# rmcolq/charon

Hardware: AMD Instinct MI355X
Metric: classified reads/sec + achieved HBM GB/s vs roofline, 5 kb reads, 39 GB index (higher is better)
Workload: dtype u64

## Files before the change

### charon_amd/csrc/charon_hip.hip

```cpp

#include <hip/hip_runtime.h>

#include <algorithm>
#include <chrono>
#include <functional>
#include <cmath>
#include <cstddef>
#include <cstdint>
#include <cstdio>
#include <cstdlib>
#include <cstring>
#include <limits>
#include <mutex>
#include <new>
#include <string>
#include <type_traits>
#include <vector>

#include "charon_hip.h"
#include "default_kde.inc"

#include "parts/common.inc"
#include "parts/k1_minimise_probe.inc"
#include "parts/k2_count_wavelog.inc"
#include "parts/shard_kernels.inc"
#include "parts/shardx_kernels.inc"
#include "parts/k3_model_call.inc"
#include "parts/len_order.inc"
#include "parts/gzip_trees.inc"
#include "parts/gzip_walk.inc"
#include "parts/gzip_tally.inc"
#include "parts/gzip_size_dev.inc"
#include "parts/gzip_tally_long.inc"
#include "parts/text_pack.inc"
#include "parts/text_split.inc"
#include "parts/fasta_split.inc"
#include "parts/text_gather.inc"
// ... 20 lines not shown
```

### charon_amd/csrc/parts/abi_shard_wait.inc

```

static int ensure_shard_buffers(chn_stream *s) {
    const uint64_t nw = (s->cfg.max_reads + WAVE - 1) / WAVE;
    int rc;
    if ((rc = s->big.ensure(s->cfg.max_bases, nw, (uint32_t)s->idx->d.bin_words, 65536, 0))) return rc;
    if ((rc = s->d_list.ensure(s->big.log_cap * 8)) || (rc = s->d_cbase.ensure((nw + 1) * 8))) return rc;
    return CHN_OK;
}
static ShardArgs shard_args(chn_stream *s, const chn_index *shard, uint64_t *partial, const Slot &sl) {
    ShardArgs a;
    std::memset(&a, 0, sizeof a);
    const chn_index_desc &d = shard->d;
    a.list = s->d_list.as<uint64_t>(); a.wave_meta = s->big.meta.as<WaveMeta>(); a.cbase = s->d_cbase.as<uint64_t>();
    a.wave_count = s->big.wcount.as<uint32_t>(); a.words = shard->words; a.S = d.bin_size; a.row_begin = d.row_begin; a.row_end = d.row_end;
    a.shift = (uint32_t)d.hash_shift; a.h = d.hash_funs; a.W = (uint32_t)d.bin_words; a.partial = partial; a.rows = s->big.rows.as<uint64_t>();
    a.rowlog = s->big.log.as<uint32_t>(); a.B = (uint32_t)d.bins;
    a.n_waves = (uint32_t)((sl.n_reads + WAVE - 1) / WAVE); a.esc_capacity = s->big.esc_cap;
    a.status = reinterpret_cast<uint32_t *>(const_cast<Slot &>(sl).d_ctl.as<unsigned long long>() + CTL_STATUS);
    return a;
}

extern "C" int chn_shard_minimise(chn_stream *s, const chn_batch *b, uint64_t *n_entries) {
    if (!s || !b || !n_entries) return fail(CHN_E_INVALID, "chn_shard_minimise: null argument");
    if (s->shard_open || s->shx_stage != 0) return fail(CHN_E_STATE, "chn_shard_minimise: previous sharded batch not finished");
    HIPCHK(hipSetDevice(s->idx->d.device));
// ... 125 lines not shown
    const chn_index_desc &d = s->idx->d;
    unsigned long long *ctl = sl.d_ctl.as<unsigned long long>();
    const uint64_t n = sl.n_reads, nw = (n + WAVE - 1) / WAVE + sl.split_bound;
    HIPCHK(hipMemsetAsync(ctl, 0, CTL_NLONG * 8, s->stream));
    HIPCHK(hipMemsetAsync(ctl + CTL_FETCHES, 0, (CTL_WORDS - CTL_FETCHES) * 8, s->stream));
    hipLaunchKernelGGL(k_sum_len, dim3((uint32_t)std::min<uint64_t>(1024, (n + 255) / 256)), dim3(256), 0, s->stream, sl.len1, sl.len2, (uint32_t)n, ctl + CTL_WORDS - 1);
    HIPCHK(hipGetLastError());
    unsigned long long total = 0;
    HIPCHK(hipMemcpyAsync(&total, ctl + CTL_WORDS - 1, 8, hipMemcpyDeviceToHost, s->stream));
    HIPCHK(hipStreamSynchronize(s->stream));
    int rc = s->big.ensure(total, (n + WAVE - 1) / WAVE + std::min<uint64_t>(sl.split_bound, total / len_bucket_floor(std::min(s->long_bucket, 247u)) + 1), (uint32_t)d.bin_words, 65536, 0, nw);
    if (rc) return rc;
    K1Args a = sl.k1;
    a.gate_started = a.gate_signal = nullptr;
    fill_k1_log(a, sl, s->big, true);
    const size_t lds = k1_lds_bytes(a.wn, d.num_categories, MODE_ROWS, a.h, (uint32_t)d.bin_words, (uint32_t)d.bins);
    hipError_t e = launch_k1_mode(MODE_ROWS, (uint32_t)d.bin_words, a, lds, s->stream);
    if (e == hipSuccess && sl.split_bound) e = launch_k1_split_mode(MODE_ROWS, (uint32_t)d.bin_words, a, lds, s->stream, split_grid(sl.split_bound));
    if (e != hipSuccess) return fail(CHN_E_HIP, std::string("k_minimise_probe re-run: ") + hipGetErrorString(e));
    if ((rc = launch_tail(s, sl, s->big, s->stream))) return rc;
    HIPCHK(hipStreamSynchronize(s->stream));
    s->overflow_reruns += 1;
    return CHN_OK;
}

extern "C" int chn_batch_wait(chn_stream *s, chn_result *r) {
    if (!s || !r || r->struct_size != sizeof(chn_result)) return fail(CHN_E_INVALID, "chn_batch_wait: bad argument");
    if (s->inflight == 0) return fail(CHN_E_STATE, "no batch in flight");
    HIPCHK(hipSetDevice(s->idx->d.device));
    Slot &sl = s->slot[(s->head + chn_stream::N_SLOTS - s->inflight) % chn_stream::N_SLOTS];
    static const bool diag_wait = diag_env("CHN_DIAG_WAIT") != nullptr;
// ... 227 lines not shown
```

### charon_amd/csrc/parts/abi_stream_batch.inc

```

struct ResLayout {
    size_t ctl, prob, nh, counts, unique, call, conf, flags, total;
    ResLayout(uint64_t n, uint64_t C) {
        ctl = 0; prob = CTL_WORDS * 8; nh = prob + n * C * 8; counts = nh + n * 4; unique = counts + n * C * 4; call = unique + n * C * 4;
        conf = call + n; flags = conf + n; total = flags + n;
    }
};

static const int PROF_ANCHOR_SECONDS = 8;
static hipError_t prof_anchor_now(chn_stream *s) {
    for (Slot &sl : s->slot) sl.new_anchor = false;
    s->prof_cur = 0; s->prof_anchor_pending = false; s->prof_have_end = false; s->prof_prev_end = 0;
    hipError_t e = hipEventRecord(s->prof_anchor[0], s->stream);
    if (e == hipSuccess) e = hipEventSynchronize(s->prof_anchor[0]);
    s->prof_anchor_at = std::chrono::steady_clock::now();
    return e;
}

extern "C" int chn_stream_create(chn_index *idx, const chn_stream_cfg *cfg, chn_stream **out) {
    if (!idx || !cfg || !out || cfg->struct_size != sizeof(chn_stream_cfg)) return fail(CHN_E_INVALID, "chn_stream_create: bad argument");
    if (cfg->max_reads == 0 || cfg->max_reads > 0xFFFFFF00ULL) return fail(CHN_E_INVALID, "max_reads out of range");
    HIPCHK(hipSetDevice(idx->d.device));
    idx->ef_release();
    chn_stream *s = new (std::nothrow) chn_stream();
// ... 183 lines not shown
    k.memo = s->d_memo.as<ulonglong2>(); k.memo_mask = memo_entries - 1;
    k.tab = s->d_model.as<uint32_t>();
    k.data = reinterpret_cast<const float *>(static_cast<char *>(s->d_model.p) + tab_bytes);
    k.C = C; k.h_pos = M.h_pos; k.h_neg = M.h_neg; k.rate = M.rate; k.log_rate = std::log(M.rate);
    k.min_quality = M.min_quality; k.min_compression = M.min_compression; k.cpt = M.cpt; k.lo_thr = M.lo_thr;
    k.min_pd = M.min_pd; k.min_prd = M.min_prd; k.min_length = M.min_length; k.conf_thr = (int32_t)M.conf_thr;
    k.min_hits = M.min_hits; k.paired = M.paired; k.host_index = M.host_index;
    k.dist = M.dist;
    k.dparams = reinterpret_cast<const float *>(static_cast<char *>(s->d_model.p) + tab_bytes + flat_bytes);
    s->k3 = k;
    s->model = std::move(M);
    s->model.set = true;
    return CHN_OK;
}

static bool k1_cond(int mode, uint32_t B) { return mode == MODE_FUSED && B <= K1_COND_MAX_BINS; }
template <int W, int MODE, bool SPLIT = false, bool COND = false>
static hipError_t launch_k1(const K1Args &a, size_t lds, hipStream_t st, uint32_t blocks = 0) {
    if (!SPLIT) blocks = (a.n_reads + WAVE - 1) / WAVE;
    if (lds > 48 * 1024) {
        hipError_t e = hipFuncSetAttribute((const void *)k_minimise_probe<W, MODE, 0, SPLIT, COND>, hipFuncAttributeMaxDynamicSharedMemorySize, (int)lds);
        if (e != hipSuccess) return e;
    }
    if (a.wn == 23)
        hipLaunchKernelGGL((k_minimise_probe<W, MODE, 23, SPLIT, COND>), dim3(blocks), dim3(WAVE), lds, st, a);
    else
        hipLaunchKernelGGL((k_minimise_probe<W, MODE, 0, SPLIT, COND>), dim3(blocks), dim3(WAVE), lds, st, a);
    return hipGetLastError();
}
static hipError_t launch_k1_split_mode(int mode, uint32_t W, const K1Args &a, size_t lds, hipStream_t st, uint32_t blocks) {
    if (mode == MODE_FUSED) return k1_cond(mode, a.B) ? launch_k1<1, MODE_FUSED, true, true>(a, lds, st, blocks) : launch_k1<1, MODE_FUSED, true, false>(a, lds, st, blocks);
    switch (W) {
        case 1: return launch_k1<1, MODE_ROWS, true>(a, lds, st, blocks);
        case 2: return launch_k1<2, MODE_ROWS, true>(a, lds, st, blocks);
        case 3: return launch_k1<3, MODE_ROWS, true>(a, lds, st, blocks);
        default: return launch_k1<4, MODE_ROWS, true>(a, lds, st, blocks);
    }
}
static uint32_t split_bound(const chn_stream *s, const Slot &sl, uint64_t n, uint64_t n_bases, bool paired) {
// ... 2 lines not shown
    (void)n_bases;
    if (!sl.host_batch) return (uint32_t)n;
    uint64_t c = 0;
    for (uint32_t L : sl.h_len1) c += L >= floor_len;
    return (uint32_t)c;
}
static uint32_t split_grid(uint32_t bound) { return std::min<uint32_t>(bound, 8192u); }
template <int MODE>
static hipError_t launch_k1_w(uint32_t W, const K1Args &a, size_t lds, hipStream_t st) {
    switch (W) {
        case 1: return launch_k1<1, MODE>(a, lds, st);
        case 2: return launch_k1<2, MODE>(a, lds, st);
        case 3: return launch_k1<3, MODE>(a, lds, st);
        default: return launch_k1<4, MODE>(a, lds, st);
    }
}
static size_t k1_lds_bytes(uint32_t wn, uint32_t C, int mode, uint32_t h, uint32_t W, uint32_t B) {
    const bool cond = k1_cond(mode, B);
    const size_t qc = cond ? QCAP + WAVE : QCAP;
    size_t b = (size_t)wn * WAVE * 8 + qc * 8 + qc * 4 + (cond ? qc * 8 : 0) + (mode == MODE_EMPLACE ? WAVE * 8 : 0) + (size_t)wn * WAVE;
    if (mode == MODE_FUSED) b += (size_t)2 * C * WAVE * 4;
    if (cond) b += (size_t)FUSED_ROUNDS * 1024;
    else if (mode == MODE_FUSED || mode == MODE_ROWS) b += (size_t)2 * h * (W <= 2 ? 1 : 2) * 1024;
    b = (b + 15) & ~(size_t)15;
    if (mode == MODE_ROWS) b += (size_t)(CHN_LOG_BATCH + 1) * WAVE * 4;
    return b;
}

static int upload(DevBuf &buf, const void *src, size_t bytes, hipStream_t st, size_t reserve = 0) {
    int rc = buf.ensure(std::max<size_t>(std::max(bytes, reserve), 16));
    if (rc) return rc;
    if (bytes) HIPCHK(hipMemcpyAsync(buf.p, src, bytes, hipMemcpyHostToDevice, st));
    return CHN_OK;
}

static int launch_tail(chn_stream *s, Slot &sl, LogBuf &lb, hipStream_t st);
static void fill_k1_log(K1Args &a, Slot &sl, LogBuf &lb, bool dynamic) {
    a.rowlog = lb.log.as<uint32_t>(); a.rows = lb.rows.as<uint64_t>(); a.wave_meta = lb.meta.as<WaveMeta>(); a.wave_count = lb.wcount.as<uint32_t>();
    a.log_capacity = lb.log_cap; a.esc_capacity = lb.esc_cap; a.cap_num = lb.cap_num; a.esc_shift = lb.esc_shift;
    a.cursor = dynamic ? sl.d_ctl.as<unsigned long long>() + CTL_LOG_CURSOR : nullptr;
}
// ... 257 lines not shown
    dt[2] = dnow();
    unsigned long long *ctl = sl.d_ctl.as<unsigned long long>();
    hipLaunchKernelGGL(k_len_hist, dim3(LEN_BLOCKS), dim3(256), 0, s->stream0, sl.len1, sl.len2, (uint32_t)n, s->d_hist.as<uint32_t>(), ctl);
    sl.split_bound = list_mode ? 0u : split_bound(s, sl, n, b->n_bases, paired);
    hipLaunchKernelGGL(k_len_scatter, dim3(LEN_BLOCKS), dim3(256), 0, s->stream0, sl.len1, sl.len2, (uint32_t)n, s->d_hist.as<uint32_t>(), sl.d_order.as<uint32_t>(),
                       ctl, sl.split_bound ? s->long_bucket : 256u, sl.split_bound);
    HIPCHK(hipGetLastError());
    HIPCHK(hipEventRecord(sl.uploaded, s->stream0));
    HIPCHK(hipStreamWaitEvent(ps, sl.uploaded, 0));

    K1Args &a = sl.k1;
    std::memset(&a, 0, sizeof(a));
    a.words = s->idx->words; a.S = d.bin_size; a.row_begin = d.row_begin; a.row_end = d.row_end; a.seed = d.minimiser_seed; a.powk1 = pow5(d.kmer_size - 1);
    a.shift = (uint32_t)d.hash_shift; a.h = d.hash_funs; a.k = d.kmer_size; a.wn = d.window_size - d.kmer_size + 1;
    a.n_reads = (uint32_t)n; a.nseg = paired ? 2 : 1; a.B = (uint32_t)d.bins; a.C = C;
    for (uint32_t bb = 0; bb < 8 && bb < d.bins; ++bb) a.b2c_packed |= (uint64_t)d.bin_to_category[bb] << (8 * bb);
    a.bases = bases; a.nmask = nmask; a.off1 = off1; a.off2 = off2; a.len1 = sl.len1; a.len2 = sl.len2; a.n_bases = b->n_bases;
    a.order = sl.d_order.as<uint32_t>();
    a.status = reinterpret_cast<uint32_t *>(ctl + CTL_STATUS);
    if (const char *ab = diag_env("CHN_ABLATE")) a.ablate = (uint32_t)std::atoi(ab);
    a.nt_probes = s->idx->rows_local * d.bin_words * 8 > (4ULL << 30) ? 1u : 0u;
    if (const char *nt = diag_env("CHN_NT_PROBES")) a.nt_probes = (uint32_t)std::atoi(nt);
    a.num_hashes = sl.d_num_hashes.as<uint32_t>(); a.counts = sl.d_counts.as<uint32_t>(); a.unique = sl.d_unique.as<uint32_t>();
    const uint32_t n_waves = (uint32_t)((n + WAVE - 1) / WAVE);
    a.n_long_ptr = sl.split_bound ? ctl + CTL_NLONG : nullptr; a.wave_slot0 = n_waves;
    a.fetches = ctl + CTL_FETCHES;
    if (list_kind == LIST_SPARSE) {
        fill_k1_log(a, sl, s->shx, true);
        a.rows = s->d_list.as<uint64_t>();
    } else if (list_mode) {
        fill_k1_log(a, sl, s->big, false);
        a.rows = s->d_list.as<uint64_t>();
        hipLaunchKernelGGL(k_wave_caps, dim3((uint32_t)((n + 255) / 256)), dim3(256), 0, ps, sl.d_order.as<uint32_t>(), sl.len1, sl.len2,
                           (uint32_t)n, s->big.cap_num, s->big.esc_shift, s->big.meta.as<WaveMeta>());
        hipLaunchKernelGGL(k_scan_meta, dim3(1), dim3(1024), 0, ps, s->big.meta.as<WaveMeta>(), n_waves);
        HIPCHK(hipGetLastError());
    } else if (!fused) {
        fill_k1_log(a, sl, sl.lb, true);
    }
    const int mode = list_mode ? MODE_LIST : fused ? MODE_FUSED : MODE_ROWS;
    size_t lds = k1_lds_bytes(a.wn, C, mode, a.h, W, a.B);
    if (const char *pad = diag_env("CHN_LDS_PAD")) lds += (size_t)std::atoi(pad);
    if (lds > 160 * 1024) return fail(CHN_E_INVALID, "window too large for LDS");
    if (sl.split_bound) {
        HIPCHK(hipStreamWaitEvent(s->stream4, sl.uploaded, 0));
        hipError_t e4 = launch_k1_split_mode(mode, W, a, lds, s->stream4, split_grid(sl.split_bound));
        if (e4 != hipSuccess) return fail(CHN_E_HIP, std::string("k_minimise_probe (split) launch: ") + hipGetErrorString(e4));
        HIPCHK(hipEventRecord(sl.split_done, s->stream4));
    }
    const bool gated = !list_mode && alternate && s->gate_signal != nullptr;
    if (gated) {
        if (s->gate_seq) {
            HIPCHK(hipStreamWaitValue64(ps, s->gate_signal, s->gate_seq, hipStreamWaitValueGte, ~0ull));
            s->gated_batches += 1;
        }
        a.gate_started = ctl + CTL_GATE; a.gate_signal = s->gate_signal; a.gate_value = s->gate_seq + 1;
// ... 38 lines not shown
    const uint32_t W = (uint32_t)d.bin_words, C = d.num_categories;
    const uint32_t n_waves = (uint32_t)((n + WAVE - 1) / WAVE);
    const bool prof = (s->cfg.flags & CHN_STREAM_PROFILE) != 0 && st == s->stream2;
    unsigned long long *ctl = sl.d_ctl.as<unsigned long long>();
    if (!sl.fused) {
        K2Args k2;
        std::memset(&k2, 0, sizeof(k2));
        k2.rows = lb.rows.as<uint64_t>(); k2.rowlog = lb.log.as<uint32_t>();
        k2.wave_meta = lb.meta.as<WaveMeta>(); k2.wave_count = lb.wcount.as<uint32_t>(); k2.order = sl.d_order.as<uint32_t>();
        k2.counts = sl.d_counts.as<uint32_t>(); k2.unique = sl.d_unique.as<uint32_t>();
        k2.n_reads = (uint32_t)n; k2.B = (uint32_t)d.bins; k2.C = C; k2.W = W;
        std::memcpy(k2.b2c, d.bin_to_category, 256);
        k2.n_long_ptr = sl.split_bound && !sl.list_mode ? ctl + CTL_NLONG : nullptr; k2.wave_slot0 = n_waves;
        const dim3 grid(n_waves), block(K2_THREADS);
        const bool t16 = !sl.list_mode && sl.len2 == nullptr && s->long_bucket <= LONG_BUCKET_DEFAULT;
        uint32_t G = WAVE;
        while (G > 8 && k2_lds_bytes((uint32_t)d.bins, C, W, G, t16) > K2_LDS_BUDGET) G >>= 1;
        k2.group = G;
        const size_t lds2 = k2_lds_bytes((uint32_t)d.bins, C, W, G, t16);
        if (lds2 > 150 * 1024) return fail(CHN_E_INVALID, "bins x categories too large for the count kernel's LDS");
        const void *fn = t16 ? (W == 1 ? (const void *)k_count_wavelog<1, true> : W == 2 ? (const void *)k_count_wavelog<2, true> : W == 3 ? (const void *)k_count_wavelog<3, true> : (const void *)k_count_wavelog<4, true>)
                             : (W == 1 ? (const void *)k_count_wavelog<1, false> : W == 2 ? (const void *)k_count_wavelog<2, false> : W == 3 ? (const void *)k_count_wavelog<3, false> : (const void *)k_count_wavelog<4, false>);
        if (lds2 > 48 * 1024) HIPCHK(hipFuncSetAttribute(fn, hipFuncAttributeMaxDynamicSharedMemorySize, (int)lds2));
        if (prof) HIPCHK(hipEventRecord(sl.ev[2], st));
        {
            void *args[] = {(void *)&k2};
            HIPCHK(hipLaunchKernel(fn, grid, block, args, lds2, st));
        }
        if (k2.n_long_ptr) {
            const dim3 lgrid(std::min<uint32_t>(sl.split_bound, 4096u)), lblock(K2L_THREADS);
            switch (W) {
                case 1: hipLaunchKernelGGL(k_count_longlog<1>, lgrid, lblock, 0, st, k2); break;
// ... 60 lines not shown
```

### charon_amd/csrc/parts/abi_synth_memory.inc

```

extern "C" int chn_synth_genomes(int device, uint64_t seed, uint64_t n_genomes, uint64_t genome_len, uint32_t **dev_bases2) {
    if (!dev_bases2 || genome_len % 64 || n_genomes == 0) return fail(CHN_E_INVALID, "chn_synth_genomes: bad argument");
    HIPCHK(hipSetDevice(device));
    const uint64_t nd = n_genomes * genome_len / 16;
    uint32_t *p = nullptr;
    HIPCHK(hipMalloc((void **)&p, nd * 4));
    hipLaunchKernelGGL(k_synth_genomes, dim3((uint32_t)std::min<uint64_t>(65535, (nd + 255) / 256)), dim3(256), 0, 0, p, nd, seed);
    HIPCHK(hipGetLastError());
    HIPCHK(hipDeviceSynchronize());
    *dev_bases2 = p;
    return CHN_OK;
}
template <int W, int NT, int U>
__global__ __launch_bounds__(256) void k_gather_roof(const uint64_t *words, uint64_t rows, uint32_t iters, uint64_t *sink) {
    extern __shared__ unsigned char roof_lds[];
    uint64_t s = (blockIdx.x * (uint64_t)blockDim.x + threadIdx.x) * 0x9E3779B97F4A7C15ULL + 1;
    uint64_t acc = 0;
    typedef unsigned long long ull2 __attribute__((ext_vector_type(2)));
    for (uint32_t it = 0; it < iters; it += U) {
        ull2 v[U];
        uint64_t v1[U];
#pragma unroll
        for (int u = 0; u < U; ++u) {
            uint64_t z = s + 0x9E3779B97F4A7C15ULL;
// ... 80 lines not shown
    HIPCHK(hipMalloc((void **)&len, n * 4));
    HIPCHK(hipMalloc((void **)&bin, n));
    std::vector<uint8_t> hb(n);
    for (uint64_t i = 0; i < n; ++i) {
        hb[i] = genome_bin[i / cpg];
        if (hb[i] >= d.bins) { (void)hipFree(off); (void)hipFree(len); (void)hipFree(bin); return fail(CHN_E_INVALID, "genome_bin out of range"); }
    }
    HIPCHK(hipMemcpy(bin, hb.data(), n, hipMemcpyHostToDevice));
    hipLaunchKernelGGL(k_chunk_layout, dim3((uint32_t)((n + 255) / 256)), dim3(256), 0, 0, n_genomes, genome_len, chunk, overlap, cpg, off, len);
    K1Args a;
    std::memset(&a, 0, sizeof(a));
    a.words = idx->words; a.words_rw = idx->words; a.S = d.bin_size; a.row_begin = d.row_begin; a.row_end = d.row_end; a.seed = d.minimiser_seed; a.powk1 = pow5(d.kmer_size - 1);
    a.shift = (uint32_t)d.hash_shift; a.h = d.hash_funs; a.k = d.kmer_size; a.wn = d.window_size - d.kmer_size + 1;
    a.n_reads = (uint32_t)n; a.nseg = 1; a.B = (uint32_t)d.bins; a.C = d.num_categories;
    a.bases = dev_bases2; a.off1 = off; a.len1 = len; a.read_bin = bin; a.n_bases = n_genomes * genome_len;
    const size_t lds = k1_lds_bytes(a.wn, d.num_categories, MODE_EMPLACE, a.h, (uint32_t)d.bin_words, (uint32_t)d.bins);
    hipError_t e = launch_k1_w<MODE_EMPLACE>((uint32_t)d.bin_words, a, lds, 0);
    if (e == hipSuccess) e = hipDeviceSynchronize();
    (void)hipFree(off); (void)hipFree(len); (void)hipFree(bin);
    if (e != hipSuccess) return fail(CHN_E_HIP, std::string("plant: ") + hipGetErrorString(e));
    return CHN_OK;
}
extern "C" int chn_synth_reads(int device, uint64_t seed, const uint32_t *dev_genomes, uint64_t n_genomes, uint64_t genome_len,
                               uint64_t first_read_id, uint64_t n_reads, uint32_t read_len_min, uint32_t read_len_max, double sub_rate, double random_fraction,
                               float mean_quality, chn_synth_reads_out *out) {
    if (!out || n_reads == 0 || read_len_min == 0 || read_len_max < read_len_min) return fail(CHN_E_INVALID, "chn_synth_reads: bad argument");
    if (n_genomes && (!dev_genomes || genome_len < read_len_max)) return fail(CHN_E_INVALID, "genomes shorter than reads");
    HIPCHK(hipSetDevice(device));
    std::memset(out, 0, sizeof(*out));
    uint64_t *d_total = nullptr;
    HIPCHK(hipMalloc((void **)&out->seg1_length, n_reads * 4));
// ... 67 lines not shown
```

### charon_amd/csrc/parts/k1_minimise_probe.inc

```

enum { MODE_FUSED = 0, MODE_ROWS = 1, MODE_EMPLACE = 2, MODE_LIST = 3 };
#ifndef CHN_LOG_BATCH
#define CHN_LOG_BATCH 4
#endif
#ifndef CHN_BASE_PIECES
#define CHN_BASE_PIECES 4
#endif

#ifndef K1_COND_MAX_BINS
#define K1_COND_MAX_BINS 4u
#endif
#ifndef FUSED_ROUNDS
#define FUSED_ROUNDS 2u
#endif

struct WaveMeta { uint64_t base, esc_base; uint32_t cap, esc_cap, pad0, pad1; };

struct K1Args {
    const uint64_t *words;
    uint64_t *words_rw;
    uint64_t S, row_begin, row_end, seed, powk1;
    uint32_t shift, h, k, wn, n_reads, nseg, B, C;
    uint64_t b2c_packed;
    const uint32_t *bases, *nmask;
// ... 1 lines not shown
    const uint32_t *len1, *len2;
    const uint32_t *order;
    uint32_t *num_hashes, *counts, *unique;
    uint64_t *rows;
    uint32_t *rowlog;
    WaveMeta *wave_meta;
    uint32_t *wave_count;
    unsigned long long *cursor;
    uint64_t log_capacity, esc_capacity;
    uint32_t cap_num, esc_shift;
    uint32_t *status;
    uint64_t n_bases;
    uint32_t nt_probes;
    const uint8_t *read_bin;
    uint32_t ablate;
    const unsigned long long *n_long_ptr;
    uint32_t wave_slot0;
    unsigned long long *fetches;
    unsigned long long *gate_started, *gate_signal;
    unsigned long long gate_value;
};
__global__ void k_gate_release(unsigned long long *signal, unsigned long long value) {
    if (threadIdx.x == 0 && blockIdx.x == 0) [[clang::atomic(remote_memory, fine_grained_memory)]] {
        (void)__hip_atomic_fetch_max(signal, value, __ATOMIC_RELAXED, __HIP_MEMORY_SCOPE_SYSTEM);
    }
}

__device__ bool first_window_tied(const K1Args &a, uint64_t o, uint32_t wn) {
    const uint64_t INV5 = 0xCCCCCCCCCCCCCCCDULL;
    const uint32_t k = a.k, w = wn + k - 1;
// ... 63 lines not shown
    switch (n) {
        case 0: asm volatile("s_waitcnt vmcnt(0)" ::: "memory"); break;
        case 1: asm volatile("s_waitcnt vmcnt(1)" ::: "memory"); break;
        case 2: asm volatile("s_waitcnt vmcnt(2)" ::: "memory"); break;
        case 3: asm volatile("s_waitcnt vmcnt(3)" ::: "memory"); break;
        case 4: asm volatile("s_waitcnt vmcnt(4)" ::: "memory"); break;
        case 5: asm volatile("s_waitcnt vmcnt(5)" ::: "memory"); break;
        case 6: asm volatile("s_waitcnt vmcnt(6)" ::: "memory"); break;
        case 7: asm volatile("s_waitcnt vmcnt(6)" ::: "memory"); break;
        case 8: asm volatile("s_waitcnt vmcnt(8)" ::: "memory"); break;
        case 9: asm volatile("s_waitcnt vmcnt(8)" ::: "memory"); break;
        default: asm volatile("s_waitcnt vmcnt(10)" ::: "memory"); break;
    }
}

template <int W, int MODE, int WN_T, bool SPLIT = false, bool COND_T = false>
__global__ __launch_bounds__(WAVE) void k_minimise_probe(const K1Args a) {
    extern __shared__ __align__(16) unsigned char smem[];
    if (!SPLIT && a.gate_started && threadIdx.x == 0) {
        if (atomicAdd(a.gate_started, 1ULL) == (unsigned long long)gridDim.x - 1) [[clang::atomic(remote_memory, fine_grained_memory)]] {
            (void)__hip_atomic_fetch_max(a.gate_signal, a.gate_value, __ATOMIC_RELAXED, __HIP_MEMORY_SCOPE_SYSTEM);
        }
    }
    const uint32_t n_long = a.n_long_ptr ? (uint32_t)__builtin_nontemporal_load(a.n_long_ptr) : 0u;
    uint32_t item = blockIdx.x;
    if (SPLIT && item >= n_long) return;
    do {
    const uint32_t wslot = SPLIT ? a.wave_slot0 + item : item;
    const uint32_t wn = WN_T ? (uint32_t)WN_T : a.wn;
    constexpr uint32_t NBLK = (W == 1 || W == 2) ? 1u : 2u;
// ... 2 lines not shown
    auto qwrap = [&](uint32_t x) -> uint32_t {
        if (!COND) return x & (QC - 1);
        x = x >= QC ? x - QC : x;
        return x >= QC ? x - QC : x;
    };
    const uint32_t pb_round = COND ? 1024u : (MODE == MODE_FUSED || MODE == MODE_ROWS) ? a.h * NBLK * 1024u : 0u;
    unsigned char *pbuf = smem;
    const uint32_t pbuf_lds = (uint32_t)(size_t)(__attribute__((address_space(3))) unsigned char *)smem;
    uint64_t *ring = reinterpret_cast<uint64_t *>(smem + (COND ? FUSED_ROUNDS : 2u) * pb_round);
    uint64_t *qv = ring + (size_t)wn * WAVE;
    uint64_t *qa = qv + QC;
    uint32_t *qm = reinterpret_cast<uint32_t *>(qa + (COND ? QC : 0u));
    uint64_t *rbase = reinterpret_cast<uint64_t *>(qm + QC);
    uint32_t *cnt = reinterpret_cast<uint32_t *>(rbase + (MODE == MODE_EMPLACE ? WAVE : 0));
    uint32_t *unq = cnt + (MODE == MODE_FUSED ? a.C * WAVE : 0);
    uint8_t *spos = reinterpret_cast<uint8_t *>(unq + (MODE == MODE_FUSED ? a.C * WAVE : 0));
    uint32_t *sbuf = reinterpret_cast<uint32_t *>(smem + (((size_t)(spos + (size_t)wn * WAVE - smem) + 15) & ~(size_t)15));

    const uint32_t lane = lane_id();
    const uint32_t g = SPLIT ? item : item * WAVE + lane;
    const bool valid = SPLIT ? true : (g < a.n_reads && g >= n_long);
    const uint32_t r = valid ? (a.order ? a.order[g] : g) : 0;
    const uint32_t own = SPLIT ? 0u : lane;
    bool cold = false;

    if (MODE == MODE_FUSED)
        for (uint32_t c = 0; c < a.C; ++c) { cnt[c * WAVE + lane] = 0; unq[c * WAVE + lane] = 0; }
    if (MODE == MODE_EMPLACE) rbase[lane] = valid ? a.read_bin[r] : 0;
    __syncthreads();

    const uint32_t k = a.k;
    const uint64_t INV5 = 0xCCCCCCCCCCCCCCCDULL;
// ... 357 lines not shown
            hist2 = (hist2 << 2) | code;
            if (kHasN) histn = (histn << 1) | nf;
            fwd = (fwd - (uint64_t)d_out * a.powk1) * 5u + d_in;
            rc = (rc - cd_out) * INV5 + (uint64_t)cd_in * a.powk1;
            if (have_value) {
                const uint32_t p = i + 1 - k;
                const uint64_t vf = fwd ^ a.seed, vr = rc ^ a.seed;
                const uint64_t v = vf < vr ? vf : vr;
                if (t == 0 || v <= pv) { pv = v; pq = p; }
                if (!kSteady && p < wn) {
                    mv = pv; q = pq;
                    emit = (p == wn - 1) && !cold;
                } else if (q + wn == p) {
                    mv = pv; q = pq;
                    if (t + 1 < wn) {
                        const uint64_t sv = ring[(t + 1) * WAVE + lane];
                        if (sv < pv) { mv = sv; q = blk - wn + spos[(t + 1) * WAVE + lane]; }
                    }
                    emit = true;
                } else if (v < mv) {
                    mv = v; q = p; emit = true;
                }
                ring[t * WAVE + lane] = v;
                if (!kSteady && i + 1 == L && p + 1 < wn) emit = true;
            }
        }
        if (have_value) {
            if (t + 1 == wn) {
                uint64_t sv = ring[(wn - 1) * WAVE + lane];
                uint32_t sp = wn - 1;
                spos[(wn - 1) * WAVE + lane] = (uint8_t)sp;
#pragma unroll
                for (int u = (int)wn - 2; u >= 1; --u) {
                    const uint64_t x = ring[u * WAVE + lane];
                    if (x < sv) { sv = x; sp = (uint32_t)u; }
                    ring[u * WAVE + lane] = sv;
                    spos[u * WAVE + lane] = (uint8_t)sp;
                }
                t = 0; blk += wn;
            } else {
                ++t;
            }
        }
        const uint64_t mask = __ballot(emit);
        if (mask) {
            const uint32_t rank = __builtin_amdgcn_mbcnt_hi((uint32_t)(mask >> 32), __builtin_amdgcn_mbcnt_lo((uint32_t)mask, 0u));
            if (emit) {
                const uint32_t pos = qwrap(qhead + qcount + rank);
                qv[pos] = mv;
                qm[pos] = own;
                ++my_emitted;
            }
// ... 6 lines not shown
    const bool fast_ok = P_hi < (1u << 22);
    auto mul_digit = [&](uint32_t d) -> uint64_t {
        uint32_t hi;
        asm("v_mul_u32_u24 %0, %1, %2" : "=v"(hi) : "v"(d), "s"(P_hi));
        return (uint64_t)d * P_lo + ((uint64_t)hi << 32);
    };
    auto times5 = [&](uint64_t x) -> uint64_t {
        uint64_t r;
        asm("v_lshl_add_u64 %0, %1, 2, %1" : "=v"(r) : "v"(x));
        return r;
    };
    auto step_fast = [&](const uint32_t i, const uint32_t j, const uint32_t cur) {
        uint64_t sv = ~0ULL;
        uint32_t sq = 0;
        if (t + 1 < wn) {
            sv = ring[(t + 1) * WAVE + lane];
            sq = blk - wn + spos[(t + 1) * WAVE + lane];
        }
        const uint32_t code = (cur >> (j * 2)) & 3u;
        const uint32_t oc = (uint32_t)(hist2 >> (2 * (k - 1))) & 3u;
        hist2 = (hist2 << 2) | code;
        const uint32_t d_in = code + (code == 3u), cd_in = (3u - code) + (code == 0u);
        const uint32_t d_out = oc + (oc == 3u), cd_out = (3u - oc) + (oc == 0u);
        const uint64_t tf = fwd - mul_digit(d_out);
        fwd = times5(tf) + d_in;
        rc = (rc - cd_out) * INV5 + mul_digit(cd_in);
        const uint32_t p = i + 1 - k;
        const uint64_t vf = fwd ^ a.seed, vr = rc ^ a.seed;
        const uint64_t v = vf < vr ? vf : vr;
        const bool newpref = t == 0 || v <= pv;
        pv = newpref ? v : pv; pq = newpref ? p : pq;
        const bool expire = q + wn == p;
        const bool use_s = sv < pv;
        const uint64_t ev = use_s ? sv : pv;
        const uint32_t eq = use_s ? sq : pq;
        const bool less = v < mv;
        const bool emit = expire || less;
        mv = expire ? ev : (less ? v : mv);
        q = expire ? eq : (less ? p : q);
        ring[t * WAVE + lane] = v;
        if (t + 1 == wn) {
            if (WN_T > 1) {
                uint64_t x[WN_T > 1 ? WN_T : 2];
#pragma unroll
                for (int u = 1; u < WN_T; ++u) x[u] = ring[u * WAVE + lane];
#pragma unroll
                for (int u = 1; u < WN_T; ++u) asm volatile("" : "+v"(x[u]));
                constexpr int LAST = WN_T > 1 ? WN_T - 1 : 1;
                uint64_t bsv = x[LAST];
                uint32_t bsp = LAST;
                spos[LAST * WAVE + lane] = (uint8_t)bsp;
#pragma unroll
                for (int u = WN_T - 2; u >= 1; --u) {
                    const bool lt = x[u] < bsv;
                    bsv = lt ? x[u] : bsv; bsp = lt ? (uint32_t)u : bsp;
                    ring[u * WAVE + lane] = bsv;
                    spos[u * WAVE + lane] = (uint8_t)bsp;
                }
            } else {
                uint64_t bsv = ring[(wn - 1) * WAVE + lane];
                uint32_t bsp = wn - 1;
                spos[(wn - 1) * WAVE + lane] = (uint8_t)bsp;
                for (int u = (int)wn - 2; u >= 1; --u) {
                    const uint64_t xx = ring[u * WAVE + lane];
                    if (xx < bsv) { bsv = xx; bsp = (uint32_t)u; }
                    ring[u * WAVE + lane] = bsv;
                    spos[u * WAVE + lane] = (uint8_t)bsp;
                }
            }
            t = 0; blk += wn;
        } else {
            ++t;
// ... 113 lines not shown
```

### charon_amd/csrc/parts/k2_count_wavelog.inc

```

struct K2Args {
    const uint64_t *rows;
    const uint32_t *rowlog;
    const WaveMeta *wave_meta;
    const uint32_t *wave_count;
    const uint32_t *order;
    uint32_t *counts, *unique;
    uint32_t n_reads, B, C, W;
    uint8_t b2c[256];
    const unsigned long long *n_long_ptr;
    uint32_t wave_slot0;
    uint32_t group;
};

#define K2_THREADS 512
#ifndef K2_LDS_BUDGET
#define K2_LDS_BUDGET 7680u
#endif
#define K2_UNROLL 4
template <int W, bool T16>
__global__ __launch_bounds__(K2_THREADS) void k_count_wavelog(const K2Args a) {
    extern __shared__ __align__(16) unsigned char smem2[];
    __builtin_amdgcn_s_setprio(3);
    const uint32_t B = a.B, C = a.C, G = a.group;
    const uint32_t TB = T16 ? (B + 1) / 2 : B;
    uint32_t *tot = reinterpret_cast<uint32_t *>(smem2);
    uint32_t *unq = tot + (size_t)G * TB;
    uint64_t *cmask = reinterpret_cast<uint64_t *>(unq + (size_t)G * C + ((G * C) & 1u));
    uint8_t *chosen = reinterpret_cast<uint8_t *>(cmask + G * W);
    __shared__ uint8_t s_b2c[256];
    const uint32_t tid = threadIdx.x, g = blockIdx.x;
    const uint32_t n_long = a.n_long_ptr ? (uint32_t)*a.n_long_ptr : 0u;
    if ((g + 1) * WAVE <= n_long) return;
// ... 151 lines not shown
            } else if (x & ROWLOG_ESC_MASK) {
                const size_t j = ((x & ROWLOG_ESC_MASK) >> 2) - 1;
#pragma unroll
                for (int w = 0; w < W; ++w) {
                    const uint64_t rw = rows[j * W + w] & cmask[w];
                    found += (uint32_t)__popcll(rw);
                    if (rw) fbin = w * 64 + (uint32_t)__ffsll((long long)rw) - 1;
                }
            }
            if (found == 1) atomicAdd(&unq[s_b2c[fbin]], 1u);
        }
        __syncthreads();
        if (tid < C) a.unique[(size_t)r * C + tid] = unq[tid];
    }
}
static size_t k2_lds_bytes(uint32_t B, uint32_t C, uint32_t W, uint32_t G, bool t16) {
    const size_t tb = t16 ? (B + 1) / 2 : B;
    return (size_t)G * tb * 4 + ((size_t)G * C + ((G * C) & 1u)) * 4 + (size_t)G * W * 8 + (size_t)G * C + 16;
}

__global__ void k_wave_caps(const uint32_t *order, const uint32_t *len1, const uint32_t *len2, uint32_t n, uint32_t cap_num, uint32_t esc_shift, WaveMeta *meta) {
    const uint32_t i = blockIdx.x * blockDim.x + threadIdx.x;
    uint32_t v = 0;
    if (i < n) { const uint32_t r = order[i]; v = len1[r] + (len2 ? len2[r] : 0u); }
    uint64_t sum = v;
    for (int o = 32; o > 0; o >>= 1) sum += (uint64_t)__shfl_xor((long long)sum, o);
    if (lane_id() == 0 && i < n) {
        const uint64_t cap = wave_log_cap(sum, cap_num);
        meta[i / WAVE].base = cap;
        meta[i / WAVE].esc_base = wave_esc_cap(cap, esc_shift);
    }
}
__global__ __launch_bounds__(1024) void k_scan_meta(WaveMeta *v, uint32_t n) {
    __shared__ uint64_t part[1024][2];
// ... 23 lines not shown
```

Measured before the change: 33.20 million.

## Pack window offsets into ring values and size count-kernel LDS from leftover CU space

The minimiser ring now stores each hashed k-mer value shifted left with its window offset in the low bits, which removes the separate per-lane position byte array (spos) and its stores in the suffix-min pass. The probe kernel's LDS footprint shrinks when packing is possible, which can let more probe blocks fit per CU. The count kernel's LDS budget is now derived from the LDS left over after packing probe blocks into a CU, rather than a fixed constant, so the group size G may grow. Correctness depends on the value-bit check (ring_pack_ok) holding. The seed top bits are restored on unpacking.

```diff
diff --git a/charon_amd/csrc/charon_hip.hip b/charon_amd/csrc/charon_hip.hip
--- a/charon_amd/csrc/charon_hip.hip
+++ b/charon_amd/csrc/charon_hip.hip
@@ -21,6 +21,7 @@
 #include "default_kde.inc"
 
 #include "parts/common.inc"
+#include "parts/lds_budget.hpp"
 #include "parts/k1_minimise_probe.inc"
 #include "parts/k2_count_wavelog.inc"
 #include "parts/shard_kernels.inc"
diff --git a/charon_amd/csrc/parts/abi_shard_wait.inc b/charon_amd/csrc/parts/abi_shard_wait.inc
--- a/charon_amd/csrc/parts/abi_shard_wait.inc
+++ b/charon_amd/csrc/parts/abi_shard_wait.inc
@@ -163,7 +163,7 @@
     K1Args a = sl.k1;
     a.gate_started = a.gate_signal = nullptr;
     fill_k1_log(a, sl, s->big, true);
-    const size_t lds = k1_lds_bytes(a.wn, d.num_categories, MODE_ROWS, a.h, (uint32_t)d.bin_words, (uint32_t)d.bins);
+    const size_t lds = k1_lds_bytes(a.wn, d.num_categories, MODE_ROWS, a.h, (uint32_t)d.bin_words, (uint32_t)d.bins, a.pack != 0);
     hipError_t e = launch_k1_mode(MODE_ROWS, (uint32_t)d.bin_words, a, lds, s->stream);
     if (e == hipSuccess && sl.split_bound) e = launch_k1_split_mode(MODE_ROWS, (uint32_t)d.bin_words, a, lds, s->stream, split_grid(sl.split_bound));
     if (e != hipSuccess) return fail(CHN_E_HIP, std::string("k_minimise_probe re-run: ") + hipGetErrorString(e));
diff --git a/charon_amd/csrc/parts/abi_stream_batch.inc b/charon_amd/csrc/parts/abi_stream_batch.inc
--- a/charon_amd/csrc/parts/abi_stream_batch.inc
+++ b/charon_amd/csrc/parts/abi_stream_batch.inc
@@ -221,7 +221,6 @@
     return CHN_OK;
 }
 
-static bool k1_cond(int mode, uint32_t B) { return mode == MODE_FUSED && B <= K1_COND_MAX_BINS; }
 template <int W, int MODE, bool SPLIT = false, bool COND = false>
 static hipError_t launch_k1(const K1Args &a, size_t lds, hipStream_t st, uint32_t blocks = 0) {
     if (!SPLIT) blocks = (a.n_reads + WAVE - 1) / WAVE;
@@ -229,7 +228,7 @@
         hipError_t e = hipFuncSetAttribute((const void *)k_minimise_probe<W, MODE, 0, SPLIT, COND>, hipFuncAttributeMaxDynamicSharedMemorySize, (int)lds);
         if (e != hipSuccess) return e;
     }
-    if (a.wn == 23)
+    if (a.wn == 23 && a.pack)
         hipLaunchKernelGGL((k_minimise_probe<W, MODE, 23, SPLIT, COND>), dim3(blocks), dim3(WAVE), lds, st, a);
     else
         hipLaunchKernelGGL((k_minimise_probe<W, MODE, 0, SPLIT, COND>), dim3(blocks), dim3(WAVE), lds, st, a);
@@ -262,17 +261,6 @@
         case 3: return launch_k1<3, MODE>(a, lds, st);
         default: return launch_k1<4, MODE>(a, lds, st);
     }
-}
-static size_t k1_lds_bytes(uint32_t wn, uint32_t C, int mode, uint32_t h, uint32_t W, uint32_t B) {
-    const bool cond = k1_cond(mode, B);
-    const size_t qc = cond ? QCAP + WAVE : QCAP;
-    size_t b = (size_t)wn * WAVE * 8 + qc * 8 + qc * 4 + (cond ? qc * 8 : 0) + (mode == MODE_EMPLACE ? WAVE * 8 : 0) + (size_t)wn * WAVE;
-    if (mode == MODE_FUSED) b += (size_t)2 * C * WAVE * 4;
-    if (cond) b += (size_t)FUSED_ROUNDS * 1024;
-    else if (mode == MODE_FUSED || mode == MODE_ROWS) b += (size_t)2 * h * (W <= 2 ? 1 : 2) * 1024;
-    b = (b + 15) & ~(size_t)15;
-    if (mode == MODE_ROWS) b += (size_t)(CHN_LOG_BATCH + 1) * WAVE * 4;
-    return b;
 }
 
 static int upload(DevBuf &buf, const void *src, size_t bytes, hipStream_t st, size_t reserve = 0) {
@@ -560,6 +548,7 @@
     a.words = s->idx->words; a.S = d.bin_size; a.row_begin = d.row_begin; a.row_end = d.row_end; a.seed = d.minimiser_seed; a.powk1 = pow5(d.kmer_size - 1);
     a.shift = (uint32_t)d.hash_shift; a.h = d.hash_funs; a.k = d.kmer_size; a.wn = d.window_size - d.kmer_size + 1;
     a.n_reads = (uint32_t)n; a.nseg = paired ? 2 : 1; a.B = (uint32_t)d.bins; a.C = C;
+    a.pack = ring_pack_ok(a.k, a.wn, a.seed) ? 1u : 0u;
     for (uint32_t bb = 0; bb < 8 && bb < d.bins; ++bb) a.b2c_packed |= (uint64_t)d.bin_to_category[bb] << (8 * bb);
     a.bases = bases; a.nmask = nmask; a.off1 = off1; a.off2 = off2; a.len1 = sl.len1; a.len2 = sl.len2; a.n_bases = b->n_bases;
     a.order = sl.d_order.as<uint32_t>();
@@ -585,7 +574,7 @@
         fill_k1_log(a, sl, sl.lb, true);
     }
     const int mode = list_mode ? MODE_LIST : fused ? MODE_FUSED : MODE_ROWS;
-    size_t lds = k1_lds_bytes(a.wn, C, mode, a.h, W, a.B);
+    size_t lds = k1_lds_bytes(a.wn, C, mode, a.h, W, a.B, a.pack != 0);
     if (const char *pad = diag_env("CHN_LDS_PAD")) lds += (size_t)std::atoi(pad);
     if (lds > 160 * 1024) return fail(CHN_E_INVALID, "window too large for LDS");
     if (sl.split_bound) {
@@ -654,8 +643,9 @@
         k2.n_long_ptr = sl.split_bound && !sl.list_mode ? ctl + CTL_NLONG : nullptr; k2.wave_slot0 = n_waves;
         const dim3 grid(n_waves), block(K2_THREADS);
         const bool t16 = !sl.list_mode && sl.len2 == nullptr && s->long_bucket <= LONG_BUCKET_DEFAULT;
-        uint32_t G = WAVE;
-        while (G > 8 && k2_lds_bytes((uint32_t)d.bins, C, W, G, t16) > K2_LDS_BUDGET) G >>= 1;
+        const uint32_t wn = d.window_size - d.kmer_size + 1;
+        const size_t probe_lds = k1_lds_bytes(wn, C, MODE_ROWS, d.hash_funs, W, (uint32_t)d.bins, ring_pack_ok(d.kmer_size, wn, d.minimiser_seed));
+        const uint32_t G = k2_group((uint32_t)d.bins, C, W, t16, k2_lds_budget(probe_lds));
         k2.group = G;
         const size_t lds2 = k2_lds_bytes((uint32_t)d.bins, C, W, G, t16);
         if (lds2 > 150 * 1024) return fail(CHN_E_INVALID, "bins x categories too large for the count kernel's LDS");
diff --git a/charon_amd/csrc/parts/abi_synth_memory.inc b/charon_amd/csrc/parts/abi_synth_memory.inc
--- a/charon_amd/csrc/parts/abi_synth_memory.inc
+++ b/charon_amd/csrc/parts/abi_synth_memory.inc
@@ -118,7 +118,8 @@
     a.shift = (uint32_t)d.hash_shift; a.h = d.hash_funs; a.k = d.kmer_size; a.wn = d.window_size - d.kmer_size + 1;
     a.n_reads = (uint32_t)n; a.nseg = 1; a.B = (uint32_t)d.bins; a.C = d.num_categories;
     a.bases = dev_bases2; a.off1 = off; a.len1 = len; a.read_bin = bin; a.n_bases = n_genomes * genome_len;
-    const size_t lds = k1_lds_bytes(a.wn, d.num_categories, MODE_EMPLACE, a.h, (uint32_t)d.bin_words, (uint32_t)d.bins);
+    a.pack = ring_pack_ok(a.k, a.wn, a.seed) ? 1u : 0u;
+    const size_t lds = k1_lds_bytes(a.wn, d.num_categories, MODE_EMPLACE, a.h, (uint32_t)d.bin_words, (uint32_t)d.bins, a.pack != 0);
     hipError_t e = launch_k1_w<MODE_EMPLACE>((uint32_t)d.bin_words, a, lds, 0);
     if (e == hipSuccess) e = hipDeviceSynchronize();
     (void)hipFree(off); (void)hipFree(len); (void)hipFree(bin);
diff --git a/charon_amd/csrc/parts/k1_minimise_probe.inc b/charon_amd/csrc/parts/k1_minimise_probe.inc
--- a/charon_amd/csrc/parts/k1_minimise_probe.inc
+++ b/charon_amd/csrc/parts/k1_minimise_probe.inc
@@ -1,5 +1,4 @@
 
-enum { MODE_FUSED = 0, MODE_ROWS = 1, MODE_EMPLACE = 2, MODE_LIST = 3 };
 #ifndef CHN_LOG_BATCH
 #define CHN_LOG_BATCH 4
 #endif
@@ -39,6 +38,7 @@
     uint32_t nt_probes;
     const uint8_t *read_bin;
     uint32_t ablate;
+    uint32_t pack;
     const unsigned long long *n_long_ptr;
     uint32_t wave_slot0;
     unsigned long long *fetches;
@@ -132,6 +132,11 @@
     }
 }
 
+__host__ __device__ constexpr uint32_t ring_pbits(uint32_t wn) {
+    uint32_t n = 0;
+    for (uint32_t x = wn - 1; x; x >>= 1) ++n;
+    return n;
+}
 template <int W, int MODE, int WN_T, bool SPLIT = false, bool COND_T = false>
 __global__ __launch_bounds__(WAVE) void k_minimise_probe(const K1Args a) {
     extern __shared__ __align__(16) unsigned char smem[];
@@ -164,8 +169,13 @@
     uint64_t *rbase = reinterpret_cast<uint64_t *>(qm + QC);
     uint32_t *cnt = reinterpret_cast<uint32_t *>(rbase + (MODE == MODE_EMPLACE ? WAVE : 0));
     uint32_t *unq = cnt + (MODE == MODE_FUSED ? a.C * WAVE : 0);
+    const bool PK = WN_T ? true : a.pack != 0;
+    constexpr uint32_t PB_T = ring_pbits(WN_T ? WN_T : 1);
+    const uint32_t pbits = WN_T ? PB_T : ring_pbits(wn);
+    const uint32_t omask = (1u << pbits) - 1u;
+    const uint64_t seed_top = pbits ? (a.seed >> (64u - pbits)) << (64u - pbits) : 0ULL;
     uint8_t *spos = reinterpret_cast<uint8_t *>(unq + (MODE == MODE_FUSED ? a.C * WAVE : 0));
-    uint32_t *sbuf = reinterpret_cast<uint32_t *>(smem + (((size_t)(spos + (size_t)wn * WAVE - smem) + 15) & ~(size_t)15));
+    uint32_t *sbuf = reinterpret_cast<uint32_t *>(smem + (((size_t)(spos + (PK ? (size_t)0 : (size_t)wn * WAVE) - smem) + 15) & ~(size_t)15));
 
     const uint32_t lane = lane_id();
     const uint32_t g = SPLIT ? item : item * WAVE + lane;
@@ -553,28 +563,37 @@
                 } else if (q + wn == p) {
                     mv = pv; q = pq;
                     if (t + 1 < wn) {
-                        const uint64_t sv = ring[(t + 1) * WAVE + lane];
-                        if (sv < pv) { mv = sv; q = blk - wn + spos[(t + 1) * WAVE + lane]; }
+                        const uint64_t sw = ring[(t + 1) * WAVE + lane];
+                        const uint64_t sv = PK ? (sw >> pbits) | seed_top : sw;
+                        if (sv < pv) { mv = sv; q = PK ? blk - 1u - ((uint32_t)sw & omask) : blk - wn + spos[(t + 1) * WAVE + lane]; }
                     }
                     emit = true;
                 } else if (v < mv) {
                     mv = v; q = p; emit = true;
                 }
-                ring[t * WAVE + lane] = v;
+                ring[t * WAVE + lane] = PK ? (v << pbits) | (uint64_t)(wn - 1u - t) : v;
                 if (!kSteady && i + 1 == L && p + 1 < wn) emit = true;
             }
         }
         if (have_value) {
             if (t + 1 == wn) {
                 uint64_t sv = ring[(wn - 1) * WAVE + lane];
-                uint32_t sp = wn - 1;
-                spos[(wn - 1) * WAVE + lane] = (uint8_t)sp;
-#pragma unroll
-                for (int u = (int)wn - 2; u >= 1; --u) {
-                    const uint64_t x = ring[u * WAVE + lane];
-                    if (x < sv) { sv = x; sp = (uint32_t)u; }
-                    ring[u * WAVE + lane] = sv;
-                    spos[u * WAVE + lane] = (uint8_t)sp;
+                if (PK) {
+                    for (int u = (int)wn - 2; u >= 1; --u) {
+                        const uint64_t x = ring[u * WAVE + lane];
+                        sv = x < sv ? x : sv;
+                        ring[u * WAVE + lane] = sv;
+                    }
+                } else {
+                    uint32_t sp = wn - 1;
+                    spos[(wn - 1) * WAVE + lane] = (uint8_t)sp;
+#pragma unroll
+                    for (int u = (int)wn - 2; u >= 1; --u) {
+                        const uint64_t x = ring[u * WAVE + lane];
+                        if (x < sv) { sv = x; sp = (uint32_t)u; }
+                        ring[u * WAVE + lane] = sv;
+                        spos[u * WAVE + lane] = (uint8_t)sp;
+                    }
                 }
                 t = 0; blk += wn;
             } else {
@@ -611,8 +630,9 @@
         uint64_t sv = ~0ULL;
         uint32_t sq = 0;
         if (t + 1 < wn) {
-            sv = ring[(t + 1) * WAVE + lane];
-            sq = blk - wn + spos[(t + 1) * WAVE + lane];
+            const uint64_t sw = ring[(t + 1) * WAVE + lane];
+            sv = PK ? (sw >> pbits) | seed_top : sw;
+            sq = PK ? blk - 1u - ((uint32_t)sw & omask) : blk - wn + spos[(t + 1) * WAVE + lane];
         }
         const uint32_t code = (cur >> (j * 2)) & 3u;
         const uint32_t oc = (uint32_t)(hist2 >> (2 * (k - 1))) & 3u;
@@ -635,7 +655,7 @@
         const bool emit = expire || less;
         mv = expire ? ev : (less ? v : mv);
         q = expire ? eq : (less ? p : q);
-        ring[t * WAVE + lane] = v;
+        ring[t * WAVE + lane] = PK ? (v << pbits) | (uint64_t)(wn - 1u - t) : v;
         if (t + 1 == wn) {
             if (WN_T > 1) {
                 uint64_t x[WN_T > 1 ? WN_T : 2];
@@ -645,14 +665,17 @@
                 for (int u = 1; u < WN_T; ++u) asm volatile("" : "+v"(x[u]));
                 constexpr int LAST = WN_T > 1 ? WN_T - 1 : 1;
                 uint64_t bsv = x[LAST];
-                uint32_t bsp = LAST;
-                spos[LAST * WAVE + lane] = (uint8_t)bsp;
 #pragma unroll
                 for (int u = WN_T - 2; u >= 1; --u) {
-                    const bool lt = x[u] < bsv;
-                    bsv = lt ? x[u] : bsv; bsp = lt ? (uint32_t)u : bsp;
+                    bsv = x[u] < bsv ? x[u] : bsv;
                     ring[u * WAVE + lane] = bsv;
-                    spos[u * WAVE + lane] = (uint8_t)bsp;
+                }
+            } else if (PK) {
+                uint64_t bsv = ring[(wn - 1) * WAVE + lane];
+                for (int u = (int)wn - 2; u >= 1; --u) {
+                    const uint64_t xx = ring[u * WAVE + lane];
+                    bsv = xx < bsv ? xx : bsv;
+                    ring[u * WAVE + lane] = bsv;
                 }
             } else {
                 uint64_t bsv = ring[(wn - 1) * WAVE + lane];
diff --git a/charon_amd/csrc/parts/k2_count_wavelog.inc b/charon_amd/csrc/parts/k2_count_wavelog.inc
--- a/charon_amd/csrc/parts/k2_count_wavelog.inc
+++ b/charon_amd/csrc/parts/k2_count_wavelog.inc
@@ -14,9 +14,6 @@
 };
 
 #define K2_THREADS 512
-#ifndef K2_LDS_BUDGET
-#define K2_LDS_BUDGET 7680u
-#endif
 #define K2_UNROLL 4
 template <int W, bool T16>
 __global__ __launch_bounds__(K2_THREADS) void k_count_wavelog(const K2Args a) {
@@ -198,10 +195,6 @@
         if (tid < C) a.unique[(size_t)r * C + tid] = unq[tid];
     }
 }
-static size_t k2_lds_bytes(uint32_t B, uint32_t C, uint32_t W, uint32_t G, bool t16) {
-    const size_t tb = t16 ? (B + 1) / 2 : B;
-    return (size_t)G * tb * 4 + ((size_t)G * C + ((G * C) & 1u)) * 4 + (size_t)G * W * 8 + (size_t)G * C + 16;
-}
 
 __global__ void k_wave_caps(const uint32_t *order, const uint32_t *len1, const uint32_t *len2, uint32_t n, uint32_t cap_num, uint32_t esc_shift, WaveMeta *meta) {
     const uint32_t i = blockIdx.x * blockDim.x + threadIdx.x;
diff --git a/charon_amd/csrc/parts/lds_budget.hpp b/charon_amd/csrc/parts/lds_budget.hpp
--- /dev/null
+++ b/charon_amd/csrc/parts/lds_budget.hpp
@@ -0,0 +1,77 @@
+#ifndef CHN_LDS_BUDGET_HPP
+#define CHN_LDS_BUDGET_HPP
+
+#include <cstddef>
+#include <cstdint>
+
+#ifndef WAVE
+#define WAVE 64
+#endif
+#ifndef QCAP
+#define QCAP 128
+#endif
+#ifndef CHN_LOG_BATCH
+#define CHN_LOG_BATCH 4
+#endif
+#ifndef K1_COND_MAX_BINS
+#define K1_COND_MAX_BINS 4u
+#endif
+#ifndef FUSED_ROUNDS
+#define FUSED_ROUNDS 2u
+#endif
+
+enum { MODE_FUSED = 0, MODE_ROWS = 1, MODE_EMPLACE = 2, MODE_LIST = 3 };
+
+static inline uint32_t bits_u64(uint64_t x) { uint32_t n = 0; while (x) { ++n; x >>= 1; } return n; }
+static inline uint64_t pow5_u64(uint32_t e) { uint64_t p = 1; while (e--) p *= 5; return p; }
+
+static inline uint32_t ring_offset_bits(uint32_t wn) { return bits_u64((uint64_t)wn - 1); }
+static inline uint32_t ring_value_bits(uint32_t k, uint64_t seed) {
+    const uint64_t a = pow5_u64(k) - 1, b = seed >> (64 - 2 * k);
+    return bits_u64(a > b ? a : b);
+}
+static inline bool ring_pack_ok(uint32_t k, uint32_t wn, uint64_t seed) { return ring_value_bits(k, seed) + ring_offset_bits(wn) <= 64; }
+
+static inline bool k1_cond(int mode, uint32_t B) { return mode == MODE_FUSED && B <= K1_COND_MAX_BINS; }
+
+static inline size_t k1_lds_bytes(uint32_t wn, uint32_t C, int mode, uint32_t h, uint32_t W, uint32_t B, bool pack) {
+    const bool cond = k1_cond(mode, B);
+    const size_t qc = cond ? QCAP + WAVE : QCAP;
+    size_t b = (size_t)wn * WAVE * 8 + qc * 8 + qc * 4 + (cond ? qc * 8 : 0) + (mode == MODE_EMPLACE ? WAVE * 8 : 0) + (pack ? 0 : (size_t)wn * WAVE);
+    if (mode == MODE_FUSED) b += (size_t)2 * C * WAVE * 4;
+    if (cond) b += (size_t)FUSED_ROUNDS * 1024;
+    else if (mode == MODE_FUSED || mode == MODE_ROWS) b += (size_t)2 * h * (W <= 2 ? 1 : 2) * 1024;
+    b = (b + 15) & ~(size_t)15;
+    if (mode == MODE_ROWS) b += (size_t)(CHN_LOG_BATCH + 1) * WAVE * 4;
+    return b;
+}
+
+static inline size_t k2_lds_bytes(uint32_t B, uint32_t C, uint32_t W, uint32_t G, bool t16) {
+    const size_t tb = t16 ? (B + 1) / 2 : B;
+    return (size_t)G * tb * 4 + ((size_t)G * C + ((G * C) & 1u)) * 4 + (size_t)G * W * 8 + (size_t)G * C + 16;
+}
+
+#define CU_LDS_BYTES 163840u
+#define LDS_GRANULE 256u
+#define K2_LDS_STATIC 256u
+#define K2_LDS_MARGIN 1024u
+#define K2_LDS_BUDGET_MIN 7680u
+static inline size_t k2_lds_budget(size_t probe_lds) {
+#ifdef K2_LDS_BUDGET
+    (void)probe_lds;
+    return K2_LDS_BUDGET;
+#else
+    size_t p = (probe_lds + LDS_GRANULE - 1) / LDS_GRANULE * LDS_GRANULE;
+    if (p == 0 || p > CU_LDS_BYTES) return K2_LDS_BUDGET_MIN;
+    const size_t left = CU_LDS_BYTES - CU_LDS_BYTES / p * p;
+    const size_t b = left > K2_LDS_MARGIN ? left - K2_LDS_MARGIN : 0;
+    return b > K2_LDS_BUDGET_MIN ? b : K2_LDS_BUDGET_MIN;
+#endif
+}
+static inline uint32_t k2_group(uint32_t B, uint32_t C, uint32_t W, bool t16, size_t budget) {
+    uint32_t G = WAVE;
+    while (G > 8 && k2_lds_bytes(B, C, W, G, t16) > budget) G >>= 1;
+    return G;
+}
+
+#endif
```

Measured after the change: 33.78 million, median of 6. 1.02x the previous value.
